# Cathoven-AI/Montreal-Forced-Aligner

Hardware: AMD Instinct MI355X
Metric: aligned utterances/sec (whole node), 10 s utts, 5k-state triphone (higher is better)
Workload: dtype f32 scores from 2-way f16-split products (3*2^-22 per term worst case), f64 path costs

## Files before the change

montreal_forced_aligner_amd/csrc/ctx.hpp:

```cpp
#pragma once
#include <hip/hip_runtime.h>

#include <cstdarg>
#include <cstdint>
#include <cstdio>
#include <cstdlib>
#include <string>
#include <vector>

#include "../../include/mfa_hip.h"

#include "dev_buf.hpp"
#include "gmm_pack.hpp"
#include "pitch_plan.hpp"

enum { MFA_K_MFCC = 0, MFA_K_CMVN = 1, MFA_K_FEATS = 2, MFA_K_GMM = 3, MFA_K_VITERBI = 4, MFA_K_RESAMPLE = 5, MFA_K_PITCH = 6, MFA_K_COMPRESS = 7,
       MFA_K_ACC_LOOKUP = 8, MFA_K_ACC_SORT = 9, MFA_K_ACC_SUMS = 10, MFA_K_ACC_REDUCE = 11, MFA_K_EQUAL_ALIGN = 12,
       MFA_K_LDA_LOOKUP = 13, MFA_K_LDA_SECOND = 14, MFA_K_LDA_CLASS = 15, MFA_K_LDA_REDUCE = 16,
       MFA_K_MLLT_LOOKUP = 17, MFA_K_MLLT_SORT = 18, MFA_K_MLLT_SUMS = 19, MFA_K_MLLT_REDUCE = 20,
       MFA_K_TREE_KEYS = 21, MFA_K_TREE_ORDER = 22, MFA_K_TREE_SUMS = 23,
       MFA_K_VAD = 24, MFA_K_UBM_SELECT = 25, MFA_K_UBM_POST = 26, MFA_K_UBM_SUMS = 27, MFA_K_UBM_REDUCE = 28,
       MFA_K_IVEC_PRUNE = 29, MFA_K_IVEC_UTT = 30, MFA_K_IVEC_SCATTER = 31, MFA_K_IVEC_PRODUCTS = 32, MFA_K_IVEC_SOLVE = 33, MFA_K_IVEC_ACC = 34,
       MFA_K_PLDA_TRANSFORM = 35, MFA_K_PLDA_PREPARE = 36, MFA_K_PLDA_SWEEP = 37, MFA_K_PLDA_MERGE = 38,
       MFA_K_CLUSTER_SYMM = 39, MFA_K_CLUSTER_DEGREE = 40, MFA_K_CLUSTER_ROUNDS = 41, MFA_K_CLUSTER_LABELS = 42,
// ... 34 lines not shown
  int k_n[MFA_K_COUNT] = {};
  std::vector<hipEvent_t> event_pool;

  mfa_mfcc_opts mfcc{};
  bool mfcc_ready = false;
  int win = 0, shift = 0, nfft = 0;
  MfaBuf d_window;
  MfaBuf d_twiddle;
  MfaBuf d_melw;
  MfaBuf d_melidx;
  int n_melw = 0;
  int mel_np_max = 1;
  MfaBuf d_dct;
  MfaBuf d_lifter;

  std::vector<MfaResampleDevicePlan> resample_plans;

  bool pitch_ready = false;
  MfaPitchHostPlan pitch;
  MfaBuf d_pitch_f;
  MfaBuf d_pitch_i;
  MfaBuf d_pitch_ws;

  bool delta_uploaded = false;

  bool gmm_ready = false;
  int dim = 0, kpad = 0, num_pdfs = 0, num_rows = 0;
  MfaBuf d_w;
  MfaBuf d_wb;
  MfaBuf d_wh;
  MfaBuf d_gch;
  MfaBuf d_fscale;
  float gmm_acc_scale = 1.0f;
  MfaBuf d_gc;
  MfaBuf d_row0;
  MfaBuf d_nblk;
  MfaBuf d_slot;
  std::vector<int32_t> h_slot, h_nblk, h_row0, h_ngauss;
  MfaBuf d_w_stats;
  MfaBuf d_nrows;
  MfaBuf d_acc_tabs;
  bool has_slot_class[5] = {false, false, false, false, false};
  bool has_single32 = false;
  int max_nblk = 1;
  bool has_multi_block = false;
  bool all_pdfs_32row = false;

  MfaBuf d_gmm_redo;
  MfaBuf d_gmm_queue;
  MfaBuf d_xsplit;
  MfaBuf d_xsplit_bad;
  bool xsplit_ready = false;
  MfaBuf d_col_row0;
  MfaBuf d_band_ranges;
  int num_cus = 0;
  void *vit_stamps = nullptr;
  void *gmm_trace = nullptr;

  MfaBuf d_ws;
  MfaBuf d_gen_ws;
  MfaBuf d_gen_list;

  int fail(const char *fmt, ...) {
    char buf[1024];
    va_list ap;
    va_start(ap, fmt);
    vsnprintf(buf, sizeof(buf), fmt, ap);
    va_end(ap);
    err = buf;
    return -1;
  }
};

#define MFA_HIP_CHECK(ctx, expr)                                                                 \
  do {                                                                                           \
    hipError_t _e = (expr);                                                                      \
    if (_e != hipSuccess) return (ctx)->fail("%s failed: %s (%s:%d)", #expr, hipGetErrorString(_e), __FILE__, __LINE__); \
  } while (0)

inline bool mfa_debug_sync_enabled() {
  static const bool on = [] { const char *e = getenv("MFA_DEBUG_SYNC"); return e && e[0] == '1'; }();
  return on;
}
#define MFA_DEBUG_POINT(ctx, ...)                                                                         \
  do {                                                                                                    \
    if (mfa_debug_sync_enabled()) {                                                                       \
      fprintf(stderr, "[mfa] " __VA_ARGS__); fprintf(stderr, "\n"); fflush(stderr);                       \
      hipError_t _e = hipStreamSynchronize((ctx)->stream);                                                \
      if (_e == hipSuccess) _e = hipGetLastError();                                                       \
      if (_e != hipSuccess) return (ctx)->fail("launch failed: %s (%s:%d)", hipGetErrorString(_e), __FILE__, __LINE__); \
    }                                                                                                     \
  } while (0)

inline int mfa_num_cus(mfa_ctx *c) {
  if (c->num_cus <= 0) {
    hipDeviceProp_t prop;
    const hipError_t e = hipGetDeviceProperties(&prop, c->device);
    if (e != hipSuccess) { c->fail("hipGetDeviceProperties failed: %s", hipGetErrorString(e)); return 0; }
    c->num_cus = prop.multiProcessorCount;
  }
  return c->num_cus;
}

inline int mfa_list_grid(mfa_ctx *c) {
  const char *e = getenv("MFA_LIST_GRID");
  const int forced = e ? atoi(e) : 0;
  return forced > 0 ? forced : 4 * mfa_num_cus(c);
}

struct KernelTimer {
  mfa_ctx *c; int which; hipEvent_t a = nullptr, b = nullptr;
  KernelTimer(mfa_ctx *ctx, int w) : c(ctx), which(w) {
    if (!c->kernel_timing) return;
    a = get(); b = get();
    (void)hipEventRecord(a, c->stream);
  }
  ~KernelTimer() {
    if (!c->kernel_timing) return;
    (void)hipEventRecord(b, c->stream);
    c->pending.push_back({which, a, b});
  }
  hipEvent_t get() {
    if (!c->event_pool.empty()) { hipEvent_t e = c->event_pool.back(); c->event_pool.pop_back(); return e; }
    hipEvent_t e = nullptr; (void)hipEventCreate(&e); return e;
  }
};

int mfa_resolve_timers(mfa_ctx *ctx);

size_t mfa_int_scan_blocks(int64_t total);
void mfa_int_scan(mfa_ctx *ctx, const int32_t *d_v, int64_t total, int32_t *d_bsum, int32_t *d_base, int32_t *d_G);

struct MfaLazyScoring {
  mfa_score_plan plan;
  const float *d_feats;
  int max_frames;
  int window;
};
struct MfaWindowScore {
  int t_begin, window;
  const int32_t *band;
  const int32_t *utt_list;
  const int32_t *n_list;
  const int32_t *done;
  int done_stride, done_word;
  const int32_t *lag;
  int lag_stride, lag_word;
  int cols_per_wave;
  int hi_slack;
};
constexpr int kMfaRunSlots = MFA_PLAN_MAX_GROUPS;
constexpr int kMfaRangeSlots = kMfaRunSlots + 5;
const int32_t *mfa_band_ranges(mfa_ctx *ctx);
int mfa_gmm_presplit(mfa_ctx *c, const MfaLazyScoring *lazy, const int64_t *d_frame_off, int n_utt, int64_t total_frames);
int mfa_gmm_lazy_supported(mfa_ctx *ctx);
int mfa_gmm_score_window(mfa_ctx *ctx, const MfaLazyScoring *lazy, const MfaWindowScore *ws, const int64_t *d_frame_off,
                         int n_utt, const int64_t *d_ll_off, float *d_loglikes);
```

montreal_forced_aligner_amd/csrc/gmm_band.hip:

```cpp
#include <algorithm>
#include <cmath>
#include <cstdint>
#include <cstdlib>
#include <cstring>
#include <type_traits>

#include "gmm_common.hpp"

namespace {

__global__ void gmm_col_rows_kernel(GmmParams p, int32_t *out) {
  const int utt = blockIdx.x;
  const int64_t l0 = p.pdf_off[utt], l1 = p.pdf_off[utt + 1];
  for (int64_t j = l0 + threadIdx.x; j < l1; j += blockDim.x) {
    const int pdf = p.pdf_list[j];
    int r = p.row0[pdf];
    if (p.col_nb_packed) { const int nb = p.nblk[pdf]; if (nb > 1) r |= nb - 1; }
    out[j] = r;
  }
}

constexpr int kRunSlots = kMfaRunSlots;
constexpr int kRangeSlots = kMfaRangeSlots;
__global__ __launch_bounds__(256) void gmm_band_ranges_kernel(GmmParams p) {
  const int lane = threadIdx.x & 63;
  const int utt = blockIdx.x * 4 + (threadIdx.x >> 6);
  if (utt >= p.n_utt) return;
  if (p.b_t_begin > 0 && p.b_done && p.b_done[(size_t)utt * p.b_done_stride + p.b_done_word] != 0) return;
  const int64_t l0 = p.pdf_off[utt];
  const int32_t *cc6 = p.class_counts + (size_t)utt * 6;
  const Band bd = band_of(p, utt);
  const int runs = p.groups > 1 ? p.groups : 1;
  int32_t *out = p.ranges + (size_t)utt * kRangeSlots * 2;
  int off = 0;
  for (int slot = 0; slot < kRangeSlots; slot++) {
    int cnt = 0, base = 0;
    if (slot < kRunSlots) {
      if (slot >= runs) continue;
      if (p.groups > 1) { const int32_t *gc = p.group_counts + (size_t)utt * p.groups; for (int g = 0; g < slot; g++) base += gc[g]; cnt = gc[slot]; }
      else cnt = cc6[0];
      off = 0;
    } else if (slot == kRunSlots + 3) {
      off = cc6[0];
      cnt = cc6[1];
    } else if (slot == kRunSlots + 4) {
      off = cc6[0] + cc6[1] + cc6[2] + cc6[3] + cc6[4];
      cnt = cc6[5];
    } else {
      const int cls = slot - kRunSlots + 2;
      off = cc6[0] + cc6[1];
      for (int k = 2; k < cls; k++) off += cc6[k];
      cnt = cc6[cls];
    }
    int nh = 0, nl = 0;
    for (int i0 = 0; i0 < cnt; i0 += 256) {
      int ff[4], ld[4];
#pragma unroll
      for (int u = 0; u < 4; u++) {
        const int i = min(i0 + 64 * u + lane, cnt - 1);
        ff[u] = p.first_frame[l0 + off + base + i]; ld[u] = p.last_depth[l0 + off + base + i];
      }
#pragma unroll
      for (int u = 0; u < 4; u++) {
        const bool in = i0 + 64 * u + lane < cnt;
        nh += __popcll(__ballot(in && ff[u] <= bd.hi));
        nl += __popcll(__ballot(in && ld[u] < bd.lo));
      }
    }
    if (lane == 0) { out[2 * slot] = base + min(nl, nh); out[2 * slot + 1] = base + nh; }
  }
}
// ... 74 lines not shown
  if constexpr (kStrided) walk = band_walk(p, wave, true);
  const int grp = kStrided ? walk.grp : (p.b_split ? band_split_block(p).y : 0);
  const bool sweep = kStrided && !kHalf && p.redo_mode == 2 && p.b_utt_list == nullptr;
  int witem = walk.first - walk.stride, blk = (walk.first - walk.stride) * 64;
  unsigned long long flagged = 0ull;
  auto next_item = [&]() -> bool {
    if (!sweep) { witem += walk.stride; return witem < walk.n_witems; }
    while (flagged == 0ull) {
      blk += walk.stride * 64;
      if (blk >= walk.n_witems) return false;
      flagged = __ballot(blk + lane < walk.n_witems && p.redo[blk + lane] != 0);
    }
    witem = blk + __ffsll((long long)flagged) - 1;
    flagged &= flagged - 1ull;
    return true;
  };
  if (kStrided && !next_item()) return;
  do {
    BandStamps stamps;
    stamps.mark(0);
    int utt, r, chunk = 0;
    if (!(kStrided ? band_witem(p, witem, utt, r, &chunk) : band_item(p, wave, utt, r, &chunk))) continue;
    const int64_t f0 = p.frame_off[utt];
    const int T = (int)(p.frame_off[utt + 1] - f0);
    const int t_base = band_t_begin(p, utt) + 64 * r;
    if (t_base >= T) continue;
    int *redo_flag = p.redo + ((size_t)utt * p.b_sub + r) * p.b_nchunk + chunk;
    if (!kHalf && p.redo_mode == 2 && *redo_flag == 0) continue;
    const int col = lane & 31, h = lane >> 5;
    const int64_t l0 = p.pdf_off[utt];
    const int P = (int)(p.pdf_off[utt + 1] - l0);
    const int32_t *list = p.pdf_list + l0;
    const int32_t *cc6 = p.class_counts + (size_t)utt * 6;
    op8 b[2][kSteps][kPieces];
    bool bad = false;
    const bool presplit = kHalf && p.xsplit != nullptr;
    if (presplit) {
      const int64_t ti = xsplit_tile_index(f0, utt, t_base >> 6);
      const uint4 *src = p.xsplit + ti * (2 * kSteps * 2 * 64) + lane;
#pragma unroll
      for (int n = 0; n < 2; n++)
#pragma unroll
        for (int s_ = 0; s_ < kSteps; s_++)
#pragma unroll
          for (int q = 0; q < kPieces; q++) {
            uint4 v;
            const volatile uint4 *a4 = src + ((n * kSteps + s_) * 2 + (q & 1)) * 64;
            v.x = a4->x; v.y = a4->y; v.z = a4->z; v.w = a4->w;
            b[n][s_][q] = __builtin_bit_cast(op8, v);
          }
      bad = p.xsplit_bad[ti] != 0;
    }
    int lo_c[5], hi_c[5], base_c[5];
    {
      const int32_t *rg = p.ranges + (size_t)utt * kRangeSlots * 2;
      int off = 0;
#pragma unroll
      for (int cls = 0; cls < 5; cls++) {
        const int slot = cls == 0 ? grp : (cls == 1 ? kRunSlots + 3 : kRunSlots + cls - 2);
        base_c[cls] = off; off += cc6[cls];
        lo_c[cls] = rg[2 * slot]; hi_c[cls] = rg[2 * slot + 1];
      }
    }
    if (p.b_chunk > 0) {
      lo_c[0] += chunk * p.b_chunk;
      hi_c[0] = min(hi_c[0], lo_c[0] + p.b_chunk);
      if (chunk != 0) { hi_c[2] = lo_c[2]; hi_c[3] = lo_c[3]; hi_c[4] = lo_c[4]; }
    }
    if (p.b_split) {
      int nb_c[5], tot = 0;
#pragma unroll
      for (int cls = 2; cls < 5; cls++) {
        const int kp = cls == 2 ? 2 : (cls == 3 ? 4 : 8);
        nb_c[cls] = (hi_c[cls] + kp - 1) / kp - lo_c[cls] / kp;
        if (lo_c[cls] >= hi_c[cls]) nb_c[cls] = 0;
        tot += nb_c[cls];
      }
      const int per = (tot + p.groups - 1) / p.groups;
      const int w0 = grp * per, w1 = min(tot, w0 + per);
      int pos = 0;
#pragma unroll
      for (int cls = 2; cls < 5; cls++) {
        const int kp = cls == 2 ? 2 : (cls == 3 ? 4 : 8);
        const int jb0 = lo_c[cls] / kp;
        const int a = jb0 + max(w0 - pos, 0), b = jb0 + min(w1 - pos, nb_c[cls]);
        pos += nb_c[cls];
        if (a >= b) hi_c[cls] = lo_c[cls];
        else { lo_c[cls] = max(lo_c[cls], a * kp); hi_c[cls] = min(hi_c[cls], b * kp); }
      }
    }
    const int step1 = p.b_split ? p.groups : (p.b_chunk > 0 ? p.b_nchunk : 1);
    const int first1 = lo_c[1] + (p.b_split ? grp : (p.b_chunk > 0 ? chunk : 0));
    const int lo = lo_c[0], hi = hi_c[0];
    if (lo >= hi && first1 >= hi_c[1] && lo_c[2] >= hi_c[2] && lo_c[3] >= hi_c[3] && lo_c[4] >= hi_c[4]) {
      if (kHalf && lane == 0) *redo_flag = 0;
      continue;
    }
    stamps.mark(1);
    if (!presplit) bad = split_features<kSteps, kPieces>(p, f0, T, t_base, col, h, b);
    stamps.mark_loads_landed(2);
    if constexpr (kHalf) {
      const bool any_bad = __ballot(bad) != 0ull;
      if (lane == 0) *redo_flag = any_bad ? 1 : 0;
      if (any_bad) continue;
    }
    const float inv_s = kHalf ? p.acc_scale_inv : 1.0f;
    const float l2e_s = 1.44269504088896341f * inv_s;
    float *out = p.out + p.ll_off[utt];
    constexpr int kProd = Ops::kProd;
    auto flush_cols = [&](int c0, int cnt) {
      __builtin_amdgcn_fence(__ATOMIC_RELEASE, "wavefront");
      __builtin_amdgcn_wave_barrier();
      __builtin_amdgcn_fence(__ATOMIC_ACQUIRE, "wavefront");
#pragma unroll 4
      for (int i = 0; i < 32; i++) {
        const int rr = h + 2 * i, t = t_base + rr;
        if (col < cnt && t < T) __builtin_nontemporal_store(stage[rr * 33 + col], &out[(size_t)t * P + c0 + col]);
      }
      __builtin_amdgcn_fence(__ATOMIC_RELEASE, "wavefront");
      __builtin_amdgcn_wave_barrier();
    };

    if (lo < hi) {
      const uint4 *wsrc = (kHalf ? p.wh : p.wb) + lane;
      const float *gsrc = (kHalf ? p.gch : p.gc) + 4 * h;
      const int last = hi - 1;
      const int32_t *crow = p.col_row0 + l0;
      auto row0_at = [&](int jj) { return crow[min(jj, last)]; };
      auto block_at = [&](int jj) {
        const int blk = __builtin_amdgcn_readfirstlane(row0_at(jj)) >> 5;
        return blk;
      };
      op8 a[kSteps][kPieces];
      f32x4 g[4];
      {
        const int blk = block_at(lo);
        const uint4 *src = wsrc + (size_t)blk * kUnits;
#pragma unroll
        for (int q = 0; q < 4; q++) g[q] = *reinterpret_cast<const f32x4 *>(gsrc + (size_t)blk * 32 + 8 * q);
#pragma unroll
        for (int s_ = 0; s_ < kSteps; s_++)
#pragma unroll
          for (int q = 0; q < kPieces; q++) a[s_][q] = __builtin_bit_cast(op8, src[(s_ * kPieces + q) * 64]);
      }
      int blk_next = block_at(lo + 1);
      for (int j = lo; j < hi; j++) {
        stamps.cycle(0);
        const int x_next2 = row0_at(j + 2);
        f32x16 init, acc[2];
#pragma unroll
        for (int rr = 0; rr < 16; rr++) init[rr] = g[rr >> 2][rr & 3];
        const uint4 *src = wsrc + (size_t)blk_next * kUnits;
        const float *gn = gsrc + (size_t)blk_next * 32;
#pragma unroll
        for (int s_ = 0; s_ < kSteps; s_++) {
#pragma unroll
          for (int t6 = 0; t6 < kProd; t6++)
#pragma unroll
            for (int n = 0; n < 2; n++) {
              const f32x16 &cin = (s_ == 0 && t6 == 0) ? init : acc[n];
              if constexpr (kHalf) acc[n] = __builtin_amdgcn_mfma_f32_32x32x16_f16(a[s_][Ops::pa(t6)], b[n][s_][Ops::pb(t6)], cin, 0, 0, 0);
              else acc[n] = __builtin_amdgcn_mfma_f32_32x32x16_bf16(a[s_][Ops::pa(t6)], b[n][s_][Ops::pb(t6)], cin, 0, 0, 0);
            }
          if (s_ == 0) {
#pragma unroll
            for (int q = 0; q < 4; q++) g[q] = *reinterpret_cast<const f32x4 *>(gn + 8 * q);
          }
#pragma unroll
          for (int q = 0; q < kPieces; q++) a[s_][q] = __builtin_bit_cast(op8, src[(s_ * kPieces + q) * 64]);
          __builtin_amdgcn_sched_barrier(0);
        }
        stamps.cycle(1);
        blk_next = __builtin_amdgcn_readfirstlane(x_next2) >> 5;
        stamps.cycle(2);
        const Lse lse0 = block_lse(acc[0], h, l2e_s), lse1 = block_lse(acc[1], h, l2e_s);
        const int jj = (j - lo) & 31;
        stage[(32 * h + col) * 33 + jj] = finish((h ? lse1.m : lse0.m) * inv_s, h ? lse1.s : lse0.s);
        stamps.cycle_lds_landed(3);
        if (jj == 31 || j == last) flush_cols(j - jj, jj + 1);
        stamps.cycle(4);
        stamps.block_done();
      }
      stamps.add_block_phases(p, lane == 0 && kHalf);
    }

    if (first1 < hi_c[1]) {
      const uint4 *wsrc = (kHalf ? p.wh : p.wb) + lane;
      const float *gsrc = (kHalf ? p.gch : p.gc) + 4 * h;
      const int32_t *crow1 = p.col_row0 + l0 + base_c[1];
      const int last1 = hi_c[1] - 1;
      auto col_word = [&](int jj) { return crow1[min(jj, last1)]; };
      auto blocks_of = [&](int word, int jj) {
        return p.col_nb_packed ? (word & 31) + 1 : __builtin_amdgcn_readfirstlane(p.nblk[list[base_c[1] + min(jj, last1)]]);
      };
      int j1 = first1;
      int word = __builtin_amdgcn_readfirstlane(col_word(j1));
      int nb = blocks_of(word, j1), blk = word >> 5, bk = 0;
      int word_n = col_word(j1 + step1);
      op8 a[kSteps][kPieces];
      f32x4 g[4];
      {
        const uint4 *src = wsrc + (size_t)blk * kUnits;
#pragma unroll
        for (int q = 0; q < 4; q++) g[q] = *reinterpret_cast<const f32x4 *>(gsrc + (size_t)blk * 32 + 8 * q);
#pragma unroll
        for (int s_ = 0; s_ < kSteps; s_++)
#pragma unroll
          for (int q = 0; q < kPieces; q++) a[s_][q] = __builtin_bit_cast(op8, src[(s_ * kPieces + q) * 64]);
      }
      float M[2] = {0.0f, 0.0f}, S[2] = {0.0f, 0.0f};
      for (;;) {
        const bool last_blk = bk + 1 == nb;
        const bool more_cols = j1 + step1 < hi_c[1];
        int blk_n = blk + 1;
        if (last_blk) blk_n = more_cols ? __builtin_amdgcn_readfirstlane(word_n) >> 5 : blk;
        f32x16 init, acc[2];
#pragma unroll
        for (int rr = 0; rr < 16; rr++) init[rr] = g[rr >> 2][rr & 3];
        const uint4 *src = wsrc + (size_t)blk_n * kUnits;
        const float *gn = gsrc + (size_t)blk_n * 32;
#pragma unroll
        for (int s_ = 0; s_ < kSteps; s_++) {
#pragma unroll
          for (int t6 = 0; t6 < kProd; t6++)
#pragma unroll
            for (int n = 0; n < 2; n++) {
              const f32x16 &cin = (s_ == 0 && t6 == 0) ? init : acc[n];
              if constexpr (kHalf) acc[n] = __builtin_amdgcn_mfma_f32_32x32x16_f16(a[s_][Ops::pa(t6)], b[n][s_][Ops::pb(t6)], cin, 0, 0, 0);
              else acc[n] = __builtin_amdgcn_mfma_f32_32x32x16_bf16(a[s_][Ops::pa(t6)], b[n][s_][Ops::pb(t6)], cin, 0, 0, 0);
            }
          if (s_ == 0) {
#pragma unroll
            for (int q = 0; q < 4; q++) g[q] = *reinterpret_cast<const f32x4 *>(gn + 8 * q);
          }
// ... 19 lines not shown
      }
    }

    auto run_small = [&](auto slot_c, int base, int lo_s, int hi_s) {
      constexpr int kSlot = decltype(slot_c)::value, kPdfs = 32 / kSlot;
      if (lo_s >= hi_s) return;
      const uint4 *wsrc = kHalf ? p.wh : p.wb;
      const float *gsrc = kHalf ? p.gch : p.gc;
      const int rho = lane & 31, my_k = rho / kSlot, my_r = rho % kSlot;
      const int jb0 = lo_s / kPdfs, jb1 = (hi_s + kPdfs - 1) / kPdfs;
      auto row_of = [&](int jb) -> int {
        const int idx = min(jb, jb1 - 1) * kPdfs + my_k;
        return idx < hi_s ? p.col_row0[l0 + base + idx] + my_r : p.num_rows;
      };
      auto src_of = [&](int row) { return wsrc + (size_t)(row >> 5) * kUnits + (row & 31) + 32 * h; };
      op8 a[kSteps][kPieces];
      int row_cur = row_of(jb0), row_next = row_of(jb0 + 1);
      float gcv = gsrc[row_cur];
      {
        const uint4 *src = src_of(row_cur);
#pragma unroll
        for (int s_ = 0; s_ < kSteps; s_++)
#pragma unroll
          for (int q = 0; q < kPieces; q++) a[s_][q] = __builtin_bit_cast(op8, src[(s_ * kPieces + q) * 64]);
      }
      const int col0 = base + jb0 * kPdfs;
      for (int jb = jb0; jb < jb1; jb++) {
        const int row_n2 = row_of(jb + 2);
        f32x16 init, acc[2];
#pragma unroll
        for (int rr = 0; rr < 16; rr++) init[rr] = __shfl(gcv, acc_row(rr, h));
        const uint4 *src = src_of(row_next);
#pragma unroll
        for (int s_ = 0; s_ < kSteps; s_++) {
#pragma unroll
          for (int t6 = 0; t6 < kProd; t6++)
#pragma unroll
            for (int n = 0; n < 2; n++) {
              const f32x16 &cin = (s_ == 0 && t6 == 0) ? init : acc[n];
              if constexpr (kHalf) acc[n] = __builtin_amdgcn_mfma_f32_32x32x16_f16(a[s_][Ops::pa(t6)], b[n][s_][Ops::pb(t6)], cin, 0, 0, 0);
              else acc[n] = __builtin_amdgcn_mfma_f32_32x32x16_bf16(a[s_][Ops::pa(t6)], b[n][s_][Ops::pb(t6)], cin, 0, 0, 0);
            }
          if (s_ == 0) gcv = gsrc[row_next];
#pragma unroll
          for (int q = 0; q < kPieces; q++) a[s_][q] = __builtin_bit_cast(op8, src[(s_ * kPieces + q) * 64]);
          __builtin_amdgcn_sched_barrier(0);
        }
        row_next = row_n2;
        small_slot_scores<kSlot>(acc, stage, col, ((jb - jb0) * kPdfs) & 31, h, inv_s, l2e_s);
        const int done = (jb - jb0 + 1) * kPdfs;
        if ((done & 31) == 0 || jb == jb1 - 1) {
          const int first = (done - 1) & ~31;
          const int valid = min(done, hi_s - jb0 * kPdfs) - first;
          flush_cols(col0 + first, valid);
        }
      }
    };
    run_small(std::integral_constant<int, 16>{}, base_c[2], lo_c[2], hi_c[2]);
    run_small(std::integral_constant<int, 8>{}, base_c[3], lo_c[3], hi_c[3]);
    run_small(std::integral_constant<int, 4>{}, base_c[4], lo_c[4], hi_c[4]);
    stamps.add_kernel_phases(p, lane == 0 && kHalf, hi - lo);
    if constexpr (kStrided) {
      __builtin_amdgcn_fence(__ATOMIC_RELEASE, "wavefront");
      __builtin_amdgcn_wave_barrier();
      __builtin_amdgcn_fence(__ATOMIC_ACQUIRE, "wavefront");
    }
  } while (kStrided && next_item());
}

}

static int col_nb_packed_for(const mfa_ctx *c) {
  const char *e = getenv("MFA_GMM_PACK_NB");
  if (e && e[0] == '0') return 0;
  return c->max_nblk <= 32 ? 1 : 0;
}

int mfa_gmm_lazy_supported(mfa_ctx *c) { return c->gmm_ready && (c->kpad == 80 || c->kpad == 96); }

int mfa_gmm_presplit(mfa_ctx *c, const MfaLazyScoring *lazy, const int64_t *d_frame_off, int n_utt, int64_t total_frames) {
  c->xsplit_ready = false;
  {
    const int64_t cols_cap = (int64_t)n_utt * std::max(1, lazy->plan.max_cols);
    if (c->d_col_row0.reserve(c, (size_t)cols_cap * sizeof(int32_t), "the score columns' row table")) return -1;
    GmmParams q;
    memset(&q, 0, sizeof(q));
    q.row0 = c->d_row0.ptr<int32_t>(); q.pdf_list = lazy->plan.d_pdf_list; q.pdf_off = lazy->plan.d_pdf_off; q.n_utt = n_utt;
    q.nblk = c->d_nblk.ptr<int32_t>(); q.col_nb_packed = col_nb_packed_for(c);
    hipLaunchKernelGGL(gmm_col_rows_kernel, dim3(n_utt), dim3(256), 0, c->stream, q, c->d_col_row0.ptr<int32_t>());
    MFA_HIP_CHECK(c, hipGetLastError());
  }
  if (!gmm_split_passes(c).f16) return 0;
  const int64_t tiles = (total_frames >> 6) + n_utt + 1;
  if (c->d_xsplit.reserve(c, (size_t)tiles * 2 * 6 * 2 * 64 * 16, "the pre-split feature operands") ||
      c->d_xsplit_bad.reserve(c, (size_t)tiles * sizeof(int), "the pre-split tiles' range flags")) return -1;
  GmmParams p;
  memset(&p, 0, sizeof(p));
  p.dim = c->dim; p.kpad = c->kpad; p.feats = lazy->d_feats; p.frame_off = d_frame_off; p.n_utt = n_utt; p.fscale = c->d_fscale.ptr<float>();
  const int tiles_per_utt = ((lazy->max_frames + 255) / 256) * 4;
  const int64_t waves = (int64_t)n_utt * tiles_per_utt;
  const dim3 grid((unsigned)((waves + 3) / 4));
  KernelTimer kt(c, MFA_K_GMM);
  gmm_with_steps(c->kpad, [&](auto steps) {
    hipLaunchKernelGGL((gmm_presplit_kernel<steps()>), grid, dim3(256), 0, c->stream, p, c->d_xsplit.ptr<uint4>(), c->d_xsplit_bad.ptr<int>(), tiles_per_utt);
  });
  MFA_HIP_CHECK(c, hipGetLastError());
  c->xsplit_ready = true;
  return 0;
}

const int32_t *mfa_band_ranges(mfa_ctx *c) { return c->d_band_ranges.ptr<int32_t>(); }

int mfa_gmm_score_window(mfa_ctx *c, const MfaLazyScoring *lazy, const MfaWindowScore *ws, const int64_t *d_frame_off,
                         int n_utt, const int64_t *d_ll_off, float *d_loglikes) {
  if (!c->gmm_ready) return c->fail("mfa_load_gmm has not been called");
  if (!mfa_gmm_lazy_supported(c)) return c->fail("lazy scoring needs a model of at most 48 dimensions");
  if (ws->window <= 0 || ws->window % 64 != 0) return c->fail("scoring window must be a multiple of 64 frames");
  GmmParams p;
  memset(&p, 0, sizeof(p));
  p.dim = c->dim; p.kpad = c->kpad; p.num_rows = c->num_rows;
  p.w = c->d_w.ptr<float>(); p.gc = c->d_gc.ptr<float>(); p.row0 = c->d_row0.ptr<int32_t>(); p.nblk = c->d_nblk.ptr<int32_t>(); p.slot = c->d_slot.ptr<int32_t>();
  p.feats = lazy->d_feats; p.frame_off = d_frame_off; p.pdf_list = lazy->plan.d_pdf_list; p.pdf_off = lazy->plan.d_pdf_off;
  p.class_counts = lazy->plan.d_class_counts; p.ll_off = d_ll_off; p.out = d_loglikes;
  p.min_log_diff = logf(1.1920928955078125e-07f);
  p.first_frame = lazy->plan.d_pdf_first_frame; p.last_depth = lazy->plan.d_pdf_last_depth;
  p.n_utt = n_utt; p.tiles = 0;
  p.acc_scale_inv = 1.0f;
  p.trace = (unsigned long long *)c->gmm_trace;
  p.b_hi_slack = ws->hi_slack > 0 ? ws->hi_slack : 0;
  p.b_mode = 1; p.b_t_begin = ws->t_begin; p.b_sub = ws->window / 64; p.b_band = ws->band;
  p.b_utt_list = ws->utt_list; p.b_n_list = ws->n_list;
  p.b_done = ws->done; p.b_done_stride = ws->done_stride; p.b_done_word = ws->done_word;
  p.b_lag = ws->lag; p.b_lag_stride = ws->lag_stride; p.b_lag_word = ws->lag_word; p.b_lag_frames = ws->window;
  const int64_t waves = (int64_t)n_utt * p.b_sub;
  const dim3 grid((unsigned)((waves + 3) / 4));
  p.groups = lazy->plan.groups > 1 && lazy->plan.d_group_counts ? lazy->plan.groups : 0;
  p.group_counts = p.groups ? lazy->plan.d_group_counts : nullptr;
  p.b_chunk = (ws->cols_per_wave > 0 && !p.groups) ? ws->cols_per_wave : 0;
  p.b_nchunk = p.b_chunk > 0 ? (lazy->plan.max_cols + p.b_chunk - 1) / p.b_chunk : 1;
  const int64_t split_waves = waves * p.b_nchunk;
  p.b_split = p.groups > 1 ? 1 : 0;
  const dim3 split_grid((unsigned)((split_waves + 3) / 4) * (unsigned)(p.b_split ? p.groups : 1));
  const GmmSplitPasses passes = gmm_split_passes(c);
  const bool list_pass = ws->utt_list != nullptr;
  const int walk = mfa_list_grid(c);
  if (walk <= 0) return -1;
  const unsigned runs = p.b_split ? (unsigned)p.groups : 1u;
  const unsigned full_per_run = std::max(1u, (unsigned)((split_waves + 3) / 4));
  const dim3 walk_grid(std::min(((unsigned)walk + runs - 1) / runs, full_per_run) * runs);
  const dim3 walk_grid_f32(std::min((unsigned)walk, std::max(1u, grid.x)));
  KernelTimer kt(c, MFA_K_GMM);
  {
    if (c->d_band_ranges.reserve(c, (size_t)n_utt * kRangeSlots * 2 * sizeof(int32_t), "the band's index ranges")) return -1;
    p.ranges = c->d_band_ranges.ptr<int32_t>();
    hipLaunchKernelGGL(gmm_band_ranges_kernel, dim3((unsigned)((n_utt + 3) / 4)), dim3(256), 0, c->stream, p);
  }
  const bool split_classes = c->has_single32 || c->has_multi_block || c->has_slot_class[1] || c->has_slot_class[2] || c->has_slot_class[3];
  if (passes.bf16 && split_classes) {
    if (c->d_gmm_redo.reserve(c, (size_t)split_waves * sizeof(int), "the scoring redo list")) return -1;
    p.redo = c->d_gmm_redo.ptr<int>();
    p.wb = c->d_wb.ptr<const uint4>();
    p.col_row0 = c->d_col_row0.ptr<int32_t>();
    p.col_nb_packed = col_nb_packed_for(c);
    if (passes.f16) {
      p.wh = c->d_wh.ptr<const uint4>(); p.gch = c->d_gch.ptr<float>(); p.fscale = c->d_fscale.ptr<float>();
      p.acc_scale_inv = 1.0f / c->gmm_acc_scale;
      p.redo_mode = 0;
      if (c->xsplit_ready) { p.xsplit = c->d_xsplit.ptr<const uint4>(); p.xsplit_bad = c->d_xsplit_bad.ptr<int>(); }
      gmm_with_steps(c->kpad, [&](auto steps) {
        if (list_pass) hipLaunchKernelGGL((gmm_band_kernel<steps(), 2, true>), walk_grid, dim3(256), 0, c->stream, p);
        else hipLaunchKernelGGL((gmm_band_kernel<steps(), 2>), split_grid, dim3(256), 0, c->stream, p);
      });
      p.redo_mode = 2;
    }
    gmm_with_steps(c->kpad, [&](auto steps) {
      if (list_pass || p.redo_mode == 2) hipLaunchKernelGGL((gmm_band_kernel<steps(), 3, true>), walk_grid, dim3(256), 0, c->stream, p);
      else hipLaunchKernelGGL((gmm_band_kernel<steps(), 3>), split_grid, dim3(256), 0, c->stream, p);
    });
    p.redo_mode = 0;
    p.b_skip0 = 1;
  }
  p.b_split = 0;
  const bool f32_classes = c->has_slot_class[4];
  if (!p.b_skip0 || f32_classes) mfa_gmm_launch_band_f32(c, &p, list_pass ? walk_grid_f32 : grid, list_pass);
  MFA_HIP_CHECK(c, hipGetLastError());
  return 0;
}
```

montreal_forced_aligner_amd/csrc/gmm_common.hpp:

```cpp
#pragma once
#include <climits>
#include <cstdint>
#include <cstdlib>
#include <type_traits>

#include "ctx.hpp"

namespace {

typedef float f32x16 __attribute__((ext_vector_type(16)));
typedef float f32x4 __attribute__((ext_vector_type(4)));
typedef __bf16 bf16x8 __attribute__((ext_vector_type(8)));
typedef _Float16 f16x8 __attribute__((ext_vector_type(8)));

struct GmmParams {
  int dim, kpad, num_rows;
  const float *w; const float *gc; const int32_t *row0; const int32_t *nblk; const int32_t *slot;
  const uint4 *wb;
  const uint4 *wh;
  const float *gch;
  const float *fscale;
  float acc_scale_inv;
  int *redo;
  int redo_mode;
  int *redo_count;
  const float *feats; const int64_t *frame_off;
  const int32_t *pdf_list; const int64_t *pdf_off; const int32_t *class_counts; const int64_t *ll_off;
  unsigned long long *trace;
  int skip_cc0;
  int skip_single;
  const int32_t *first_frame;
  float *out;
  float min_log_diff;
  int n_utt, tiles;
  int *queue;
  const int *max_ff;
  int b_mode;
  int b_t_begin, b_sub;
  const int32_t *b_band;
  const int32_t *b_utt_list; const int32_t *b_n_list;
  const int32_t *b_done; int b_done_stride, b_done_word;
  const int32_t *b_lag; int b_lag_stride, b_lag_word, b_lag_frames;
  const int32_t *last_depth;
  int b_skip0;
  int b_chunk, b_nchunk;
  const uint4 *xsplit;
  const int *xsplit_bad;
  const int32_t *col_row0;
  int32_t *ranges;
  int groups;
  const int32_t *group_counts;
  int b_split;
  int b_hi_slack;
  int col_nb_packed;
};

struct Band { int lo, hi; };
__device__ __forceinline__ int band_lag(const GmmParams &p, int utt) {
  return (p.b_lag && p.b_t_begin > 0) ? (p.b_lag[(size_t)utt * p.b_lag_stride + p.b_lag_word] != 0 ? 1 : 0) : 0;
}
__device__ __forceinline__ int band_t_begin(const GmmParams &p, int utt) { return p.b_t_begin - band_lag(p, utt) * p.b_lag_frames; }
__device__ __forceinline__ Band band_of(const GmmParams &p, int utt) {
  Band b;
  const int lag = band_lag(p, utt);
  if (p.b_t_begin - lag * p.b_lag_frames <= 0) { b.lo = 0; b.hi = 64 * p.b_sub - 1; }
  else { b.lo = p.b_band[2 * utt]; b.hi = p.b_band[2 * utt + 1]; }
  if (p.b_hi_slack > 0 && !lag && b.hi != INT32_MAX) b.hi -= p.b_hi_slack;
  return b;
}
__device__ __forceinline__ int2 band_split_block(const GmmParams &p) {
  if (p.groups <= 8) return make_int2((int)(blockIdx.x / (unsigned)p.groups), (int)(blockIdx.x % (unsigned)p.groups));
  const unsigned half = gridDim.x >> 1, phase = blockIdx.x >= half ? 1u : 0u, rem = blockIdx.x - phase * half;
  return make_int2((int)(rem >> 3), (int)(phase * 8u + (rem & 7u)));
}
__device__ __forceinline__ bool band_witem(const GmmParams &p, int witem, int &utt, int &r, int *chunk = nullptr) {
  if (chunk) { const int q = witem / p.b_nchunk; *chunk = witem - q * p.b_nchunk; witem = q; }
  const int item = witem / p.b_sub;
  r = witem - item * p.b_sub;
  const int n_items = p.b_n_list ? *p.b_n_list : p.n_utt;
  if (item >= n_items) return false;
  utt = p.b_utt_list ? p.b_utt_list[item] : item;
  if (p.b_t_begin > 0 && p.b_done && p.b_done[(size_t)utt * p.b_done_stride + p.b_done_word] != 0) return false;
  return true;
}
__device__ __forceinline__ bool band_item(const GmmParams &p, int wave, int &utt, int &r, int *chunk = nullptr) {
  return band_witem(p, (p.b_split ? band_split_block(p).x : (int)blockIdx.x) * 4 + wave, utt, r, chunk);
}
struct BandWalk { int first, stride, n_witems, grp; };
__device__ __forceinline__ BandWalk band_walk(const GmmParams &p, int wave, bool chunks) {
  BandWalk w;
  const unsigned runs = p.b_split ? (unsigned)p.groups : 1u;
  w.grp = (int)(blockIdx.x % runs);
  w.first = (int)(blockIdx.x / runs) * 4 + wave;
  w.stride = (int)(gridDim.x / runs) * 4;
  const int n_items = p.b_n_list ? *p.b_n_list : p.n_utt;
  w.n_witems = n_items * p.b_sub * (chunks ? p.b_nchunk : 1);
  return w;
}

__device__ __forceinline__ int prefix_end(unsigned long long mask, int i0) { return mask ? i0 + 64 - __clzll((long long)mask) : 0; }

// ... 235 lines not shown
```

montreal_forced_aligner_amd/csrc/viterbi.hip:

```cpp
#include <cstdlib>
#include <cstring>

#include <algorithm>
#include <vector>

#include "viterbi_common.hpp"
#include "viterbi_wave.hpp"
#include "viterbi_small.hpp"
#include "viterbi_plan.hpp"

namespace {

__global__ void collect_pending_kernel(const int32_t *status, int n_utt, int code, int32_t *list, int32_t *count) {
  const int i = blockIdx.x * blockDim.x + threadIdx.x;
  if (i < n_utt && status[i] == code) list[atomicAdd(count, 1)] = i;
}
__global__ void finalize_pending_kernel(int32_t *status, int n_utt) {
  const int i = blockIdx.x * blockDim.x + threadIdx.x;
  if (i < n_utt && status[i] == ST_PENDING) status[i] = ST_FAILED;
}

__global__ void arcnext_kernel(mfa_graph_batch g, uint4 *out, u32 *epsinfo, int max_states) {
  const int utt = blockIdx.x;
  const int64_t so = g.d_state_off[utt], ab = g.d_arc_base[utt];
// ... 46 lines not shown
}

extern "C" {

MFA_API int mfa_debug_viterbi_stamps(mfa_ctx *c, void *d_stamps) {
  c->vit_stamps = d_stamps;
  return 0;
}

MFA_API int mfa_debug_viterbi_plan(const mfa_align_opts *o, int32_t max_states, int32_t max_arcs, int32_t eps, int32_t lazy,
                                   int32_t *h_out, int32_t cap) {
  return vplan::viterbi_plan_rows(o, max_states, max_arcs, eps != 0, lazy != 0, h_out, cap);
}

MFA_API size_t mfa_align_workspace_bytes(mfa_ctx *c, int32_t n_utt, int64_t total_frames, const mfa_align_opts *o) {
  (void)c;
  int N = (o->max_tokens > 0 ? o->max_tokens : 1024) * 4, C = 8 * N;
  return ws_layout(n_utt, total_frames, N, C, o->bp_tokens_per_frame > 0 ? o->bp_tokens_per_frame : 512,
                   (int64_t)n_utt * 8 * N).total;
}

}

namespace {

int align_impl(mfa_ctx *c, const mfa_graph_batch *g, const float *d_loglikes, const int64_t *d_ll_off,
               const int32_t *d_ll_cols, const int64_t *d_frame_off, int64_t total_frames,
               int64_t total_arcs, int32_t max_states, int32_t max_arcs, const mfa_align_opts *o, int32_t *d_ali, int32_t *d_words, int32_t *d_n_words,
               float *d_like, float *d_frame_like, int32_t *d_status, const MfaLazyScoring *lazy) {
  MFA_HIP_CHECK(c, hipSetDevice(c->device));
  const int n_utt = g->n_utt;
  if (n_utt <= 0) return 0;
  if (o->beam <= 0.0f || (o->retry_beam != 0.0f && o->retry_beam <= o->beam))
    return c->fail("Beams do not make sense: beam %f, retry-beam %f", o->beam, o->retry_beam);
  if (max_states <= 0 || max_arcs <= 0) return c->fail("max_states and max_arcs must be positive");
  if (total_frames <= 0 || total_arcs <= 0) return c->fail("total_frames and total_arcs must be positive");
  if (max_arcs >= (1 << 25)) return c->fail("graphs with more than 2^25 arcs are not supported");
  const int bpf = o->bp_tokens_per_frame > 0 ? o->bp_tokens_per_frame : 512;
  const int passes = o->retry_beam != 0.0f ? 2 : 1;
  const bool eps = g->d_state_nemit != nullptr;
  if (eps && max_arcs >= (1 << 24)) return c->fail("graphs with epsilon arcs and more than 2^24 arcs are not supported");
  const int64_t eps_states = eps ? (int64_t)n_utt * max_states : 0;
  vplan::Plan plan = vplan::viterbi_plan(o, max_states, max_arcs, eps, lazy != nullptr);
  if (plan.refused >= 0) {
    const vplan::Launch &L = plan.l[plan.refused];
    return c->fail("Viterbi tables need %zu bytes of LDS (> 160 KiB): %d states, %d tokens", L.lds, max_states, L.N);
  }
  const int Nw = passes == 2 ? plan.N[1] : plan.N[0], Cw = passes == 2 ? plan.C[1] : plan.C[0];
  WsLayout w = ws_layout(n_utt, total_frames, Nw, Cw, bpf, total_arcs, eps_states);
  if (c->d_ws.reserve(c, w.total, "the decoder workspace")) return -1;
  unsigned char *base = c->d_ws.ptr<unsigned char>();
  hipLaunchKernelGGL(arcnext_kernel, dim3(n_utt), dim3(256), 0, c->stream, *g, (uint4 *)(base + w.arcnext),
                     eps ? (u32 *)(base + w.eps) : (u32 *)nullptr, max_states);
  if (lazy && mfa_gmm_presplit(c, lazy, d_frame_off, n_utt, total_frames) != 0) return -1;
  int spec_slack = 0;
  if (lazy) {
    int look = lazy->window / 2;
    { const char *e = getenv("MFA_LAZY_LOOKAHEAD"); if (e && atoi(e) > 0) look = atoi(e); }
    spec_slack = std::max(0, lazy->window - 1 - look);
    if (lazy->plan.max_cols > 32 * kBmWords) spec_slack = 0;
  }
  int eps_pops_env = 0;
  { const char *e = getenv("MFA_VIT_EPS_POPS"); if (e && atoi(e) > 0) eps_pops_env = atoi(e); }
  for (int li = 0; li < plan.n; li++) {
    const vplan::Launch &L = plan.l[li];
    const int ps = L.pass;
    const bool small_tier = lazy && L.grow;
    const bool lists_in_lds = L.lists_in_lds;
    const size_t lds = L.lds;
    VitParams p;
    memset(&p, 0, sizeof(p));
    p.g = *g; p.ll = d_loglikes; p.ll_off = d_ll_off; p.ll_cols = d_ll_cols; p.frame_off = d_frame_off;
    p.beam = ps == 0 ? o->beam : o->retry_beam; p.scale = o->acoustic_scale;
    p.nmax = L.N; p.cmax = L.C; p.bpf = bpf; p.pass = ps; p.grow = L.grow; p.hbits = L.hbits;
    WsLayout wp = ws_layout(n_utt, total_frames, L.N, L.C, bpf, total_arcs, eps_states);
    p.w_state = (u32 *)(base + wp.state); p.w_cost = (double *)(base + wp.cost);
    p.w_stash_a = (u32 *)(base + wp.sta); p.w_stash_b = (u32 *)(base + wp.stb); p.w_stash_key = (u64 *)(base + wp.stkey);
    p.w_bp = (u64 *)(base + wp.bp); p.w_tokoff = (u32 *)(base + wp.tokoff);
    p.w_hash = (u32 *)(base + w.hash);
    p.w_arcnext = (const uint4 *)(base + w.arcnext);
    p.w_epsinfo = eps ? (const u32 *)(base + w.eps) : nullptr; p.eps_stride = max_states;
    p.eps_pops = eps_pops_env ? eps_pops_env : 64 * L.N;
    p.llcap = kLlCap;
    p.stamps = (unsigned long long *)c->vit_stamps;
    p.utt_list = nullptr; p.n_list = nullptr;
    p.ali = d_ali; p.words = d_words; p.n_words = d_n_words; p.like = d_like; p.frame_like = d_frame_like; p.status = d_status;
    if (L.code != 0) {
      int32_t *d_list = (int32_t *)(base + w.list), *d_count = (int32_t *)(base + w.count);
      MFA_HIP_CHECK(c, hipMemsetAsync(d_count, 0, sizeof(int32_t), c->stream));
      hipLaunchKernelGGL(collect_pending_kernel, dim3((n_utt + 255) / 256), dim3(256), 0, c->stream, d_status, n_utt, L.code, d_list, d_count);
      p.utt_list = d_list; p.n_list = d_count;
    }
    p.windowed = 0; p.t_begin = 0; p.t_end = 0x7fffffff; p.next_window = 0;
    p.w_vstate = (VitState *)(base + w.vstate); p.state_depth = nullptr; p.band = nullptr;
    void (*k_lds)(VitParams) = eps ? viterbi_kernel<true, true> : viterbi_kernel<true, false>;
    void (*k_hbm)(VitParams) = eps ? viterbi_kernel<false, true> : viterbi_kernel<false, false>;
    MFA_HIP_CHECK(c, hipFuncSetAttribute((const void *)(lists_in_lds ? k_lds : k_hbm), hipFuncAttributeMaxDynamicSharedMemorySize, (int)lds));
    auto launch_decoder = [&]() {
      KernelTimer kt(c, MFA_K_VITERBI);
      if (lists_in_lds) hipLaunchKernelGGL(k_lds, dim3(n_utt), dim3(64), lds, c->stream, p);
      else hipLaunchKernelGGL(k_hbm, dim3(n_utt), dim3(64), lds, c->stream, p);
    };
    if (!lazy) {
      launch_decoder();
      MFA_DEBUG_POINT(c, "decoded pass=%d code=%d N=%d C=%d lds=%zu in_lds=%d", ps, L.code, L.N, L.C, lds, (int)lists_in_lds);
    } else {
      const int K = L.code == 0 ? lazy->window : std::max(lazy->window, 256);
// ... 80 lines not shown
```

Before: 277,500.

## Skip scoring columns whose states end before the band and dedupe shared GMM blocks

A new per-utterance kernel records, for each score column, the deepest graph state that uses it. The lazy band scorer reads this to skip columns whose owning states all lie before the current band's low edge. Within each 32-column window it scores each distinct GMM block only once and copies the result to the other columns that share it. Columns are now walked by ballot masks instead of sequentially. The cost is an extra presplit kernel, ballot and readlane overhead per window, and partial flushes with masked stores.

```diff
diff --git a/montreal_forced_aligner_amd/csrc/ctx.hpp b/montreal_forced_aligner_amd/csrc/ctx.hpp
--- a/montreal_forced_aligner_amd/csrc/ctx.hpp
+++ b/montreal_forced_aligner_amd/csrc/ctx.hpp
@@ -110,6 +110,7 @@
   MfaBuf d_xsplit_bad;
   bool xsplit_ready = false;
   MfaBuf d_col_row0;
+  MfaBuf d_col_own_last;
   MfaBuf d_band_ranges;
   int num_cus = 0;
   void *vit_stamps = nullptr;
@@ -210,7 +211,8 @@
 constexpr int kMfaRunSlots = MFA_PLAN_MAX_GROUPS;
 constexpr int kMfaRangeSlots = kMfaRunSlots + 5;
 const int32_t *mfa_band_ranges(mfa_ctx *ctx);
-int mfa_gmm_presplit(mfa_ctx *c, const MfaLazyScoring *lazy, const int64_t *d_frame_off, int n_utt, int64_t total_frames);
+int mfa_gmm_presplit(mfa_ctx *c, const MfaLazyScoring *lazy, const mfa_graph_batch *g, const int64_t *d_frame_off, int n_utt,
+                     int64_t total_frames);
 int mfa_gmm_lazy_supported(mfa_ctx *ctx);
 int mfa_gmm_score_window(mfa_ctx *ctx, const MfaLazyScoring *lazy, const MfaWindowScore *ws, const int64_t *d_frame_off,
                          int n_utt, const int64_t *d_ll_off, float *d_loglikes);
diff --git a/montreal_forced_aligner_amd/csrc/gmm_band.hip b/montreal_forced_aligner_amd/csrc/gmm_band.hip
--- a/montreal_forced_aligner_amd/csrc/gmm_band.hip
+++ b/montreal_forced_aligner_amd/csrc/gmm_band.hip
@@ -17,6 +17,26 @@
     int r = p.row0[pdf];
     if (p.col_nb_packed) { const int nb = p.nblk[pdf]; if (nb > 1) r |= nb - 1; }
     out[j] = r;
+  }
+}
+
+__global__ void gmm_col_own_last_kernel(mfa_graph_batch g, const int32_t *state_depth, const int64_t *pdf_off, int32_t *out) {
+  const int utt = blockIdx.x;
+  const int64_t l0 = pdf_off[utt];
+  const int P = (int)(pdf_off[utt + 1] - l0);
+  for (int j = threadIdx.x; j < P; j += blockDim.x) out[l0 + j] = 0;
+  __syncthreads();
+  const int64_t so = g.d_state_off[utt], ab = g.d_arc_base[utt];
+  const int S = (int)(g.d_state_off[utt + 1] - so);
+  const int32_t *arc_off = g.d_arc_off + so + utt;
+  const int32_t *nemit = g.d_state_nemit ? g.d_state_nemit + so : nullptr;
+  for (int s_ = threadIdx.x; s_ < S; s_ += blockDim.x) {
+    const int d = state_depth[2 * (so + s_)];
+    const int a0 = arc_off[s_], a1 = nemit ? a0 + nemit[s_] : arc_off[s_ + 1];
+    for (int a = a0; a < a1; a++) {
+      const int c = g.d_arc_col[ab + a];
+      if ((unsigned)c < (unsigned)P) atomicMax(&out[l0 + c], d);
+    }
   }
 }
 
@@ -197,6 +217,7 @@
       bad = p.xsplit_bad[ti] != 0;
     }
     int lo_c[5], hi_c[5], base_c[5];
+    const int band_lo = band_of(p, utt).lo;
     {
       const int32_t *rg = p.ranges + (size_t)utt * kRangeSlots * 2;
       int off = 0;
@@ -253,33 +274,49 @@
     const float l2e_s = 1.44269504088896341f * inv_s;
     float *out = p.out + p.ll_off[utt];
     constexpr int kProd = Ops::kProd;
-    auto flush_cols = [&](int c0, int cnt) {
+    auto flush_cols = [&](int c0, uint32_t cols) {
       __builtin_amdgcn_fence(__ATOMIC_RELEASE, "wavefront");
       __builtin_amdgcn_wave_barrier();
       __builtin_amdgcn_fence(__ATOMIC_ACQUIRE, "wavefront");
+      const bool mine = ((cols >> col) & 1u) != 0u;
 #pragma unroll 4
       for (int i = 0; i < 32; i++) {
         const int rr = h + 2 * i, t = t_base + rr;
-        if (col < cnt && t < T) __builtin_nontemporal_store(stage[rr * 33 + col], &out[(size_t)t * P + c0 + col]);
+        if (mine && t < T) __builtin_nontemporal_store(stage[rr * 33 + col], &out[(size_t)t * P + c0 + col]);
       }
       __builtin_amdgcn_fence(__ATOMIC_RELEASE, "wavefront");
       __builtin_amdgcn_wave_barrier();
     };
 
+    int blocks0 = 0;
     if (lo < hi) {
       const uint4 *wsrc = (kHalf ? p.wh : p.wb) + lane;
       const float *gsrc = (kHalf ? p.gch : p.gc) + 4 * h;
       const int last = hi - 1;
       const int32_t *crow = p.col_row0 + l0;
-      auto row0_at = [&](int jj) { return crow[min(jj, last)]; };
-      auto block_at = [&](int jj) {
-        const int blk = __builtin_amdgcn_readfirstlane(row0_at(jj)) >> 5;
-        return blk;
+      const int32_t *cown = p.col_own_last + l0;
+      auto win_words = [&](int j0, int &rw, int &ol) {
+        const int idx = min(j0 + col, last);
+        rw = crow[idx]; ol = cown[idx];
       };
+      auto win_masks = [&](int j0, int rw, int ol, int &first, uint32_t &need) -> uint32_t {
+        need = (uint32_t)__ballot(lane < hi - j0 && lane < 32 && ol >= band_lo);
+        first = col;
+        for (uint32_t m = need; m != 0u; m &= m - 1u) {
+          const int k = __builtin_ctz(m);
+          if (__builtin_amdgcn_readlane(rw, k) == rw && k < first) first = k;
+        }
+        return (uint32_t)__ballot(lane < 32 && ((need >> col) & 1u) != 0u && first == col);
+      };
+      int j0 = lo, rw, ol, first;
+      uint32_t need, uniq;
+      win_words(j0, rw, ol);
+      uniq = win_masks(j0, rw, ol, first, need);
+      while (uniq == 0u && j0 + 32 < hi) { j0 += 32; win_words(j0, rw, ol); uniq = win_masks(j0, rw, ol, first, need); }
       op8 a[kSteps][kPieces];
       f32x4 g[4];
-      {
-        const int blk = block_at(lo);
+      if (uniq != 0u) {
+        const int blk = __builtin_amdgcn_readlane(rw, __builtin_ctz(uniq)) >> 5;
         const uint4 *src = wsrc + (size_t)blk * kUnits;
 #pragma unroll
         for (int q = 0; q < 4; q++) g[q] = *reinterpret_cast<const f32x4 *>(gsrc + (size_t)blk * 32 + 8 * q);
@@ -288,10 +325,25 @@
 #pragma unroll
           for (int q = 0; q < kPieces; q++) a[s_][q] = __builtin_bit_cast(op8, src[(s_ * kPieces + q) * 64]);
       }
-      int blk_next = block_at(lo + 1);
-      for (int j = lo; j < hi; j++) {
+      while (uniq != 0u) {
+        int j0_n = j0 + 32, rw_n, ol_n, first_n = 0;
+        uint32_t need_n = 0u, uniq_n = 0u;
+        win_words(j0_n, rw_n, ol_n);
+        uint32_t rest = uniq;
+        blocks0 += __builtin_popcount(uniq);
+        do {
         stamps.cycle(0);
-        const int x_next2 = row0_at(j + 2);
+        const int c = __builtin_ctz(rest);
+        rest &= rest - 1u;
+        int blk_next;
+        if (rest != 0u) blk_next = __builtin_amdgcn_readlane(rw, __builtin_ctz(rest)) >> 5;
+        else {
+          if (j0_n < hi) {
+            uniq_n = win_masks(j0_n, rw_n, ol_n, first_n, need_n);
+            while (uniq_n == 0u && j0_n + 32 < hi) { j0_n += 32; win_words(j0_n, rw_n, ol_n); uniq_n = win_masks(j0_n, rw_n, ol_n, first_n, need_n); }
+          }
+          blk_next = (uniq_n != 0u ? __builtin_amdgcn_readlane(rw_n, __builtin_ctz(uniq_n)) : __builtin_amdgcn_readlane(rw, c)) >> 5;
+        }
         f32x16 init, acc[2];
 #pragma unroll
         for (int rr = 0; rr < 16; rr++) init[rr] = g[rr >> 2][rr & 3];
@@ -316,15 +368,21 @@
           __builtin_amdgcn_sched_barrier(0);
         }
         stamps.cycle(1);
-        blk_next = __builtin_amdgcn_readfirstlane(x_next2) >> 5;
         stamps.cycle(2);
         const Lse lse0 = block_lse(acc[0], h, l2e_s), lse1 = block_lse(acc[1], h, l2e_s);
-        const int jj = (j - lo) & 31;
-        stage[(32 * h + col) * 33 + jj] = finish((h ? lse1.m : lse0.m) * inv_s, h ? lse1.s : lse0.s);
+        stage[(32 * h + col) * 33 + c] = finish((h ? lse1.m : lse0.m) * inv_s, h ? lse1.s : lse0.s);
         stamps.cycle_lds_landed(3);
-        if (jj == 31 || j == last) flush_cols(j - jj, jj + 1);
+        if (rest == 0u) {
+          for (uint32_t m = need & ~uniq; m != 0u; m &= m - 1u) {
+            const int k = __builtin_ctz(m);
+            stage[lane * 33 + k] = stage[lane * 33 + __builtin_amdgcn_readlane(first, k)];
+          }
+          flush_cols(j0, need);
+        }
         stamps.cycle(4);
         stamps.block_done();
+        } while (rest != 0u);
+        j0 = j0_n; rw = rw_n; first = first_n; need = need_n; uniq = uniq_n;
       }
       stamps.add_block_phases(p, lane == 0 && kHalf);
     }
@@ -450,14 +508,14 @@
         if ((done & 31) == 0 || jb == jb1 - 1) {
           const int first = (done - 1) & ~31;
           const int valid = min(done, hi_s - jb0 * kPdfs) - first;
-          flush_cols(col0 + first, valid);
+          flush_cols(col0 + first, valid >= 32 ? ~0u : (1u << valid) - 1u);
         }
       }
     };
     run_small(std::integral_constant<int, 16>{}, base_c[2], lo_c[2], hi_c[2]);
     run_small(std::integral_constant<int, 8>{}, base_c[3], lo_c[3], hi_c[3]);
     run_small(std::integral_constant<int, 4>{}, base_c[4], lo_c[4], hi_c[4]);
-    stamps.add_kernel_phases(p, lane == 0 && kHalf, hi - lo);
+    stamps.add_kernel_phases(p, lane == 0 && kHalf, blocks0);
     if constexpr (kStrided) {
       __builtin_amdgcn_fence(__ATOMIC_RELEASE, "wavefront");
       __builtin_amdgcn_wave_barrier();
@@ -476,11 +534,15 @@
 
 int mfa_gmm_lazy_supported(mfa_ctx *c) { return c->gmm_ready && (c->kpad == 80 || c->kpad == 96); }
 
-int mfa_gmm_presplit(mfa_ctx *c, const MfaLazyScoring *lazy, const int64_t *d_frame_off, int n_utt, int64_t total_frames) {
+int mfa_gmm_presplit(mfa_ctx *c, const MfaLazyScoring *lazy, const mfa_graph_batch *g, const int64_t *d_frame_off, int n_utt,
+                     int64_t total_frames) {
   c->xsplit_ready = false;
   {
     const int64_t cols_cap = (int64_t)n_utt * std::max(1, lazy->plan.max_cols);
     if (c->d_col_row0.reserve(c, (size_t)cols_cap * sizeof(int32_t), "the score columns' row table")) return -1;
+    if (c->d_col_own_last.reserve(c, (size_t)cols_cap * sizeof(int32_t), "the score columns' own last depths")) return -1;
+    hipLaunchKernelGGL(gmm_col_own_last_kernel, dim3(n_utt), dim3(256), 0, c->stream, *g, lazy->plan.d_state_depth, lazy->plan.d_pdf_off,
+                       c->d_col_own_last.ptr<int32_t>());
     GmmParams q;
     memset(&q, 0, sizeof(q));
     q.row0 = c->d_row0.ptr<int32_t>(); q.pdf_list = lazy->plan.d_pdf_list; q.pdf_off = lazy->plan.d_pdf_off; q.n_utt = n_utt;
@@ -558,7 +620,7 @@
     if (c->d_gmm_redo.reserve(c, (size_t)split_waves * sizeof(int), "the scoring redo list")) return -1;
     p.redo = c->d_gmm_redo.ptr<int>();
     p.wb = c->d_wb.ptr<const uint4>();
-    p.col_row0 = c->d_col_row0.ptr<int32_t>();
+    p.col_row0 = c->d_col_row0.ptr<int32_t>(); p.col_own_last = c->d_col_own_last.ptr<int32_t>();
     p.col_nb_packed = col_nb_packed_for(c);
     if (passes.f16) {
       p.wh = c->d_wh.ptr<const uint4>(); p.gch = c->d_gch.ptr<float>(); p.fscale = c->d_fscale.ptr<float>();
diff --git a/montreal_forced_aligner_amd/csrc/gmm_common.hpp b/montreal_forced_aligner_amd/csrc/gmm_common.hpp
--- a/montreal_forced_aligner_amd/csrc/gmm_common.hpp
+++ b/montreal_forced_aligner_amd/csrc/gmm_common.hpp
@@ -47,6 +47,7 @@
   const uint4 *xsplit;
   const int *xsplit_bad;
   const int32_t *col_row0;
+  const int32_t *col_own_last;
   int32_t *ranges;
   int groups;
   const int32_t *group_counts;
diff --git a/montreal_forced_aligner_amd/csrc/viterbi.hip b/montreal_forced_aligner_amd/csrc/viterbi.hip
--- a/montreal_forced_aligner_amd/csrc/viterbi.hip
+++ b/montreal_forced_aligner_amd/csrc/viterbi.hip
@@ -122,7 +122,7 @@
   unsigned char *base = c->d_ws.ptr<unsigned char>();
   hipLaunchKernelGGL(arcnext_kernel, dim3(n_utt), dim3(256), 0, c->stream, *g, (uint4 *)(base + w.arcnext),
                      eps ? (u32 *)(base + w.eps) : (u32 *)nullptr, max_states);
-  if (lazy && mfa_gmm_presplit(c, lazy, d_frame_off, n_utt, total_frames) != 0) return -1;
+  if (lazy && mfa_gmm_presplit(c, lazy, g, d_frame_off, n_utt, total_frames) != 0) return -1;
   int spec_slack = 0;
   if (lazy) {
     int look = lazy->window / 2;
```

After: 294,000, median of 6. 1.06x the previous value.
